# landonclark97/numbotics

Measured on AMD Instinct MI355X. Metric: collision-checked configs/sec, Kinova 7-DoF + obstacles, higher is better.
Workload: dtype f64

## Files before the change

numbotics_amd/csrc/nbk_bf32_spec.hpp:

```cpp

#ifdef NBK_SPEC_NO_ALIGNED
#define NBK_SPEC_ALIGNED 0
#else
#define NBK_SPEC_ALIGNED 1
#endif
#ifdef NBK_SPEC_NO_QREG
#define NBK_SPEC_QREG 0
#else
#define NBK_SPEC_QREG 1
#endif
#ifdef NBK_SPEC_DIAG_NO_WORLD
#define NBK_SPEC_WORLD 0
#else
#define NBK_SPEC_WORLD 1
#endif
#ifdef NBK_SPEC_DIAG_NO_RR
#define NBK_SPEC_RR 0
#else
#define NBK_SPEC_RR 1
#endif
#ifdef NBK_SPEC_DIAG_NO_ENQUEUE
#define NBK_SPEC_ENQUEUE 0
#else
#define NBK_SPEC_ENQUEUE 1
#endif

#define NBK_SPEC_DEV __device__ __forceinline__
#define NBK_SPEC_INLINE __attribute__((always_inline))

namespace nbk_spec {

using namespace nbk;
enum { K_BOX = 2, K_HULL = 4, K_PLANE = 5 };
enum { JK_PRISMATIC = 4 };

template <int V> struct IC { static constexpr int value = V; };
template <int B, int E, class F> NBK_SPEC_DEV void sfor(F&& f) {
    if constexpr (B < E) { f(IC<B>{}); sfor<B + 1, E>(f); }
}

template <class Spec> struct SpecRoute {
    const int* __restrict__ vp_cls;
    NBK_SPEC_DEV int cls(unsigned p) const { return vp_cls[p]; }
    NBK_SPEC_DEV int base(int c) const { return Spec::cls_base[c]; }
    NBK_SPEC_DEV int groups(int c) const { return Spec::cls_groups[c]; }
};

template <class Spec>
NBK_SPEC_DEV void broad_f32_spec(const double* __restrict__ q, long long B, const float* __restrict__ ftb, const float* __restrict__ tab,
                                 unsigned long long* __restrict__ mask_bits, unsigned char* __restrict__ mask_bytes,
                                 unsigned long long* __restrict__ q_count, unsigned long long* __restrict__ q_items, unsigned long long cap,
                                 unsigned char* ovf, const int* __restrict__ vp_cls) {
    constexpr int S = Spec::S, SB = Spec::SB, NQ = Spec::NQ, J = Spec::J, W = Spec::W;
    constexpr FTabOffsets FO = ftab_offsets(W);
    extern __shared__ double lds[];
    const int lane = threadIdx.x;
    const long long base = (long long)blockIdx.x * WAVE;
    double* lds_raw = lds;
    constexpr int qrows = NQ > (SB + 2) / 2 ? NQ : (SB + 2) / 2;
    constexpr int qcap = qrows * (WAVE * 2);
    static_assert(qcap >= BQ_CAP && qcap >= S * WAVE, "the q slab must hold the general stage's queue and one unrolled block's items");
    unsigned* lds_queue = reinterpret_cast<unsigned*>(lds_raw);
    if (base >= B) return;
    const int rows_i = (int)((B - base) < WAVE ? (B - base) : WAVE);
    const bool active = lane < rows_i;
    constexpr bool QREG = NBK_SPEC_QREG != 0 && NQ <= 8;
    double qd[QREG ? NQ : 1];
    if constexpr (QREG) {
        const double* row = q + (base + (active ? lane : 0)) * NQ;
#pragma unroll
        for (int j = 0; j < NQ; ++j) qd[j] = row[j];
    } else {
        stage_plain_rows(q, base, rows_i, NQ, lds_raw, lane);
        __syncthreads();
    }
    auto qat = [&](int j) NBK_SPEC_INLINE { if constexpr (QREG) return qd[j]; else return lds_raw[lane * NQ + j]; };
    int hit = 0;
#pragma unroll
    for (int j = 0; j < NQ; ++j) hit = hit || !(__builtin_fabs(qat(j)) <= 1.7976931348623157e308);
    float cxa[SB], cya[SB], cza[SB];
#pragma unroll
    for (int i = 0; i < SB; ++i) { cxa[i] = 0.0f; cya[i] = 0.0f; cza[i] = 0.0f; }
    float rmax = Spec::f_reach, qabs = 0.0f;
    float qv[J];
#pragma unroll
    for (int k = 0; k < J; ++k) { qv[k] = (float)qat(Spec::qcol[k]); qabs += __builtin_fabsf(qv[k]); }
    XfP T;
    {
        const float* bp = ftb + Spec::f_base;
#pragma unroll
        for (int k = 0; k < 3; ++k) { T.Rc[k] = V2f{bp[k], bp[4 + k]}; T.R2[k] = bp[8 + k]; }
        T.tc = V2f{bp[3], bp[7]}; T.t2 = bp[11];
    }
    auto shapes = [&](auto K) NBK_SPEC_INLINE {
        constexpr int k = decltype(K)::value;
        sfor<Spec::sh_begin[k], Spec::sh_begin[k + 1]>([&](auto SH) NBK_SPEC_INLINE {
            constexpr int sh = decltype(SH)::value;
            const float tl0 = ftb[Spec::f_tl + 3 * sh], tl1 = ftb[Spec::f_tl + 3 * sh + 1], tl2 = ftb[Spec::f_tl + 3 * sh + 2];
            const V2f cp = fma2(T.Rc[2], splat2(tl2), fma2(T.Rc[1], splat2(tl1), fma2(T.Rc[0], splat2(tl0), T.tc)));
            const float c2 = __builtin_fmaf(T.R2[2], tl2, __builtin_fmaf(T.R2[1], tl1, __builtin_fmaf(T.R2[0], tl0, T.t2)));
            cxa[sh] = cp.x; cya[sh] = cp.y; cza[sh] = c2;
            rmax = __builtin_fmaxf(rmax, __builtin_fmaxf(__builtin_fabsf(cp.x), __builtin_fmaxf(__builtin_fabsf(cp.y), __builtin_fabsf(c2))));
        });
    };
    shapes(IC<0>{});
    sfor<0, J>([&](auto K) NBK_SPEC_INLINE {
        constexpr int k = decltype(K)::value;
        constexpr int kind = Spec::jkind[k];
        float s = 0.0f, c = 0.0f;
        if constexpr (kind != JK_PRISMATIC) sincos_f(qv[k], s, c);
        if constexpr (kind <= 2) {
            const JPk jp = *reinterpret_cast<const JPk*>(ftb + Spec::f_pk + 20 * k);
            joint_apply_axis_p<kind>(jp, T, s, c, T);
        } else {
            joint_apply_gen_p(ftb + Spec::f_rot + 27 * k, ftb + Spec::f_trans + 3 * k, ftb + Spec::f_slide + 3 * k, T, qv[k], s, c, T);
        }
        shapes(IC<k + 1>{});
    });
    const float e2 = 2.0f * rmax * __builtin_fmaf(2.4e-7f, qabs, Spec::f_eps);
    if constexpr (!QREG) __syncthreads();
    int qn = 0;
    const SpecRoute<Spec> route{vp_cls};
    const float* wbx_all = tab + FO.wbx;
    if (__builtin_amdgcn_ballot_w64(!(e2 <= Spec::f_e2max)) == 0ull) {
        sfor<0, NBK_SPEC_WORLD ? Spec::NW : 0>([&](auto WI) NBK_SPEC_INLINE {
            constexpr int wi = decltype(WI)::value;
            constexpr int w = Spec::wl[wi];
            constexpr int wk = Spec::wk[wi];
            const float* wc = ftb + Spec::f_wc + 18 * w;
            if constexpr (wk == K_BOX || wk == K_HULL) {
                const float* wb = wbx_all + w * 96;
                const float* ob = ftb + Spec::f_wobb + 6 * w;
                int cwv[SB];
                int acc_c = 0, acc_h = 0;
                sfor<0, SB / 2>([&](auto I) NBK_SPEC_INLINE {
                    constexpr int i = decltype(I)::value;
                    cwv[2 * i] = 0; cwv[2 * i + 1] = 0;
                    if constexpr (Spec::wpair(wi, 2 * i) >= 0 || Spec::wpair(wi, 2 * i + 1) >= 0) {
                        const V2f dx = V2f{cxa[2 * i], cxa[2 * i + 1]} - splat2(wc[0]);
                        const V2f dy = V2f{cya[2 * i], cya[2 * i + 1]} - splat2(wc[1]);
                        const V2f dz = V2f{cza[2 * i], cza[2 * i + 1]} - splat2(wc[2]);
                        V2i cand, certh;
                        if constexpr (wk == K_BOX) box_slot2<NBK_SPEC_ALIGNED != 0 && Spec::wbox_aligned[wi] != 0>(dx, dy, dz, wc, wb + 12 * i, cand, certh);
                        else hull_slot2(dx, dy, dz, wc, ob, wb + 12 * i, cand, certh);
                        cwv[2 * i] = cand.x; cwv[2 * i + 1] = cand.y;
                        acc_c |= cand.x | cand.y;
                        acc_h |= certh.x | certh.y;
                    }
                });
                hit = hit || (acc_h < 0);
                const bool live = active && !hit;
                if (NBK_SPEC_ENQUEUE && __builtin_amdgcn_ballot_w64(acc_c < 0 && live) != 0ull) {
                    queue_room(S * WAVE, qcap, route, lds_queue, qn, base, q_count, q_items, cap, lane, ovf);
                    sfor<0, S>([&](auto A) NBK_SPEC_INLINE {
                        constexpr int a = decltype(A)::value;
                        if constexpr (Spec::wpair(wi, a) >= 0) enqueue_lanes(cwv[a] < 0 && live, (unsigned)Spec::wpair(wi, a), lds_queue, qn, lane);
                    });
                }
            } else {
                const Row16f wkey2r = *reinterpret_cast<const Row16f*>(tab + FO.wkey2 + w * 16);
                const Row16f wcertr = *reinterpret_cast<const Row16f*>(tab + FO.wcert + w * 16);
                const Row16f wkeyr = *reinterpret_cast<const Row16f*>(tab + FO.wkey + w * 16);
                const int* tab_wp = reinterpret_cast<const int*>(tab + FO.wp);
                bool c[SB];
                bool ch = false, anyc = false;
                sfor<0, S>([&](auto A) NBK_SPEC_INLINE {
                    constexpr int a = decltype(A)::value;
                    c[a] = false;
                    if constexpr (Spec::wpair(wi, a) >= 0) {
                        if constexpr (wk == K_PLANE) {
                            if (tab_wp[w * 16 + a] >= 0) plane_slot1(cxa[a] - wc[0], cya[a] - wc[1], cza[a] - wc[2], wc, wkey2r.v[a], wcertr.v[a], c[a], ch);
                        } else {
                            if (wkeyr.v[a] >= 0.0f) sphere_slot1(cxa[a] - wc[0], cya[a] - wc[1], cza[a] - wc[2], wkey2r.v[a], wcertr.v[a], c[a], ch);
                        }
                        anyc = anyc || c[a];
                    }
                });
                hit = hit || ch;
                const bool live = active && !hit;
                if (NBK_SPEC_ENQUEUE && __builtin_amdgcn_ballot_w64(anyc && live) != 0ull) {
                    queue_room(S * WAVE, qcap, route, lds_queue, qn, base, q_count, q_items, cap, lane, ovf);
                    sfor<0, S>([&](auto A) NBK_SPEC_INLINE {
                        constexpr int a = decltype(A)::value;
                        if constexpr (Spec::wpair(wi, a) >= 0) enqueue_lanes(c[a] && live, (unsigned)Spec::wpair(wi, a), lds_queue, qn, lane);
                    });
                }
            }
        });
        if constexpr (Spec::rr_any && NBK_SPEC_RR != 0) {
            sfor<0, S - 1>([&](auto A) NBK_SPEC_INLINE {
                constexpr int a = decltype(A)::value;
                if constexpr (Spec::row_slots(a) > 0) {
                    const Row16f nk = *reinterpret_cast<const Row16f*>(tab + FO.rneg + a * 16);
                    const V2f ax2 = V2f{cxa[a], cxa[a]}, ay2 = V2f{cya[a], cya[a]}, az2 = V2f{cza[a], cza[a]};
                    V2f ev[SB / 2];
                    int acc_e = 0;
                    sfor<(a + 1) / 2, SB / 2>([&](auto I) NBK_SPEC_INLINE {
                        constexpr int i = decltype(I)::value;
                        if constexpr (Spec::rr_group(a, i)) {
                            ev[i] = slot_e2(ax2 - V2f{cxa[2 * i], cxa[2 * i + 1]}, ay2 - V2f{cya[2 * i], cya[2 * i + 1]},
                                            az2 - V2f{cza[2 * i], cza[2 * i + 1]}, V2f{nk.v[2 * i], nk.v[2 * i + 1]});
                            const V2i ei = __builtin_bit_cast(V2i, ev[i]);
                            acc_e |= ei.x | ei.y;
                        }
                    });
                    if (__builtin_amdgcn_ballot_w64(acc_e < 0 && active && !hit) != 0ull) {
                        const Row16f nd = *reinterpret_cast<const Row16f*>(tab + FO.rnd + a * 16);
                        int acc_f = 0;
                        sfor<(a + 1) / 2, SB / 2>([&](auto I) NBK_SPEC_INLINE {
                            constexpr int i = decltype(I)::value;
                            if constexpr (Spec::rr_group(a, i)) {
                                const V2i fi = __builtin_bit_cast(V2i, ev[i] + V2f{nd.v[2 * i], nd.v[2 * i + 1]});
                                acc_f |= fi.x | fi.y;
                            }
                        });
                        hit = hit || (acc_f < 0);
                        const bool live = active && !hit;
                        if (NBK_SPEC_ENQUEUE) queue_room(Spec::row_slots(a) * WAVE, qcap, route, lds_queue, qn, base, q_count, q_items, cap, lane, ovf);
                        sfor<NBK_SPEC_ENQUEUE ? a + 1 : S, S>([&](auto Bb) NBK_SPEC_INLINE {
                            constexpr int b = decltype(Bb)::value;
                            if constexpr (Spec::rr_p(a, b) >= 0) {
                                const V2i ei = __builtin_bit_cast(V2i, ev[b / 2]);
                                enqueue_lanes(((b % 2) ? ei.y : ei.x) < 0 && live, (unsigned)Spec::rr_p(a, b), lds_queue, qn, lane);
                            }
                        });
                    }
                }
            });
        }
    } else {
        const bool cert_ok = e2 <= Spec::f_e2max;
        bool certh = false;
        const float* tab_wkey = tab + FO.wkey; const float* tab_wtc = tab + FO.wtc; const float* tab_wcert = tab + FO.wcert;
        const float* tab_wcin = tab + FO.wcin; const float* tab_rho = tab + FO.rho;
        const int* tab_wp = reinterpret_cast<const int*>(tab + FO.wp);
        const int* tab_rp = reinterpret_cast<const int*>(tab + FO.rp);
        const float* tab_rkey = tab + FO.rkey; const float* tab_rcert = tab + FO.rcert;
        sfor<0, Spec::NW>([&](auto WI) NBK_SPEC_INLINE {
            constexpr int wi = decltype(WI)::value;
            constexpr int w = Spec::wl[wi];
            constexpr int wk = Spec::wk[wi];
            const float* wc = ftb + Spec::f_wc + 18 * w;
            unsigned long long bits = 0ull;
            sfor<0, S>([&](auto A) NBK_SPEC_INLINE {
                constexpr int a = decltype(A)::value;
                if constexpr (Spec::wpair(wi, a) >= 0) {
                    const float dx = cxa[a] - wc[0], dy = cya[a] - wc[1], dz = cza[a] - wc[2];
                    if constexpr (wk == K_PLANE) {
                        if (tab_wp[w * 16 + a] >= 0)
                            bits |= plane_slot_gen(dx, dy, dz, wc, tab_wkey[w * 16 + a], tab_rho[a], e2, tab_wcert[w * 16 + a], certh) ? (1ull << a) : 0ull;
                    } else if constexpr (wk == K_BOX) {
                        if (tab_wkey[w * 16 + a] >= 0.0f)
                            bits |= box_slot_gen(dx, dy, dz, wc, tab_wkey[w * 16 + a], tab_wtc[w * 16 + a], tab_rho[a], e2, tab_wcin[w * 16 + a],
                                                 certh, hit) ? (1ull << a) : 0ull;
                    } else {
                        if (tab_wkey[w * 16 + a] >= 0.0f)
                            bits |= other_slot_gen(dx, dy, dz, wc, ftb + Spec::f_wobb + 6 * w, wk == K_HULL, tab_wkey[w * 16 + a], tab_wtc[w * 16 + a],
                                                   tab_rho[a], e2, tab_wcert[w * 16 + a], certh) ? (1ull << a) : 0ull;
                    }
                }
            });
            hit = hit || (cert_ok && certh);
            if (!active || hit) bits = 0ull;
            drain_bits(bits, PairTab{tab_wp + w * 16}, route, lds_queue, qn, base, q_count, q_items, cap, lane, ovf);
        });
        if constexpr (Spec::rr_any) {
            sfor<0, S - 1>([&](auto A) NBK_SPEC_INLINE {
                constexpr int a = decltype(A)::value;
                unsigned long long bits = 0ull;
                sfor<a + 1, S>([&](auto Bb) NBK_SPEC_INLINE {
                    constexpr int b = decltype(Bb)::value;
                    if constexpr (Spec::rr_p(a, b) >= 0) {
                        bits |= robot_slot_gen(cxa[a] - cxa[b], cya[a] - cya[b], cza[a] - cza[b], tab_rkey[a * 16 + b], e2, tab_rcert[a * 16 + b], certh)
                                    ? (1ull << b) : 0ull;
                    }
                });
                hit = hit || (cert_ok && certh);
                if (!active || hit) bits = 0ull;
                drain_bits(bits, PairTab{tab_rp + a * 16}, route, lds_queue, qn, base, q_count, q_items, cap, lane, ovf);
            });
        }
    }
    if (qn > 0) flush_items_r(route, lds_queue, qn, base, q_count, q_items, cap, lane, ovf);
    write_mask(hit != 0, active, base, lane, mask_bits, mask_bytes);
}

}

#ifndef NBK_SPEC_WAVES
#define NBK_SPEC_WAVES 5
#endif
extern "C" __global__ __launch_bounds__(64, NBK_SPEC_WAVES) void k_broad_f32_spec(
        const double* __restrict__ q, long long B, const float* __restrict__ ftb, const float* __restrict__ tab,
        unsigned long long* __restrict__ mask_bits, unsigned char* __restrict__ mask_bytes, unsigned long long* __restrict__ q_count,
        unsigned long long* __restrict__ q_items, unsigned long long cap, unsigned char* ovf, const int* __restrict__ vp_cls) {
    nbk_spec::broad_f32_spec<Spec>(q, B, ftb, tab, mask_bits, mask_bytes, q_count, q_items, cap, ovf, vp_cls);
}
```

numbotics_amd/csrc/nbk_tables.hpp:

```cpp
#pragma once

namespace nbk {

enum : unsigned {
    D_JOINTS = 1,
    D_CHAIN = 2,
    D_RSHAPES = 4,
    D_WSHAPES = 8,
    D_HULL_VERTS = 16,
    D_HULL_PLANES = 32,
    D_PAIRS = 64,
    D_MOTION = D_JOINTS | D_RSHAPES | D_HULL_VERTS | D_PAIRS,
    D_ALL = 127
};

static int32_t desc_check(const nbk_model_desc* d, unsigned parts) {
    if (d == nullptr) return NBK_ERR_INVALID;
    const int J = d->n_joints, S = d->n_rshapes, W = d->n_wshapes, P = d->n_pairs, H = d->n_hulls;
    if (d->n_q < 0 || J < 0 || S < 0 || W < 0 || P < 0 || H < 0) return NBK_ERR_INVALID;
    if (J > NBK_MAX_JOINTS || d->n_q > NBK_MAX_DOF) return NBK_ERR_UNSUPPORTED;
    if (parts & D_HULL_PLANES) parts |= D_HULL_VERTS;
    if ((parts & D_HULL_VERTS) && H > 0) {
        if (d->hull_vert_begin == nullptr || d->hull_verts == nullptr || d->hull_vert_begin[0] != 0) return NBK_ERR_INVALID;
        for (int h = 0; h < H; ++h) if (d->hull_vert_begin[h + 1] <= d->hull_vert_begin[h]) return NBK_ERR_INVALID;
// ... 178 lines not shown
        else if (par < 0) t.load[k] = -1;
        else {
            if (t.save[par] < 0) t.save[par] = t.slots++;
            t.load[k] = t.save[par];
        }
    }
}

static void order_shapes(const nbk_model_desc* d, ModelTables& t) {
    const int J = d->n_joints, S = d->n_rshapes, W = d->n_wshapes;
    t.begin.assign(J + 2, 0);
    for (int f = -1; f < J; ++f) {
        t.begin[f + 1] = (int)t.order.size();
        for (int s = 0; s < S; ++s) if (d->rshape_frame[s] == f) t.order.push_back(s);
    }
    t.begin[J + 1] = (int)t.order.size();
    t.rs_kind.assign(S, 0); t.rs_row.assign(S, 0);
    t.rs_local.assign(12 * (size_t)S, 0.0); t.rs_core.assign(6 * (size_t)S, 0.0);
    t.rs_hull.assign(S > 0 ? S : 1, -1); t.ws_hull.assign(W > 0 ? W : 1, -1);
    t.rs_frame.assign(S > 0 ? S : 1, -1); t.rs_mask.assign(S > 0 ? S : 1, 0u);
    t.frame_mask = frame_masks(d);
    for (int i = 0; i < S; ++i) {
        const int s = t.order[i];
        int kind;
        robot_core_host(d, s, kind, &t.rs_core[6 * i]);
        if (kind == K_HULL) t.rs_hull[i] = (int)d->rshape_param[4 * s];
        t.rs_kind[i] = kind;
        t.rs_row[i] = t.rows;
        t.rows += host_core_rows(kind);
        memcpy(&t.rs_local[12 * i], d->rshape_local + 12 * s, 12 * sizeof(double));
        t.rs_frame[i] = d->rshape_frame[s];
        t.rs_mask[i] = t.rs_frame[i] >= 0 ? t.frame_mask[t.rs_frame[i]] : 0u;
    }
    t.ws_kind.assign(W, 0); t.ws_core.assign(18 * (size_t)W, 0.0); t.ws_center.assign(3 * (size_t)W, 0.0);
    for (int w = 0; w < W; ++w) {
        double cc[6];  int kind;
        core_params(d->wshape_type[w], d->wshape_param + 4 * w, kind, cc);
        cc[5] = 0.0;
        if (kind == K_HULL) {
            const int h = (int)d->wshape_param[4 * w];
            cc[5] = hull_bound_radius(d->hull_verts + 3 * (size_t)d->hull_vert_begin[h], d->hull_vert_begin[h + 1] - d->hull_vert_begin[h]);
            t.ws_hull[w] = h;
        }
        t.ws_kind[w] = kind;
        t.world_hulls = t.world_hulls || kind == K_HULL;
        const double* T = d->wshape_pose + 12 * w;
        double* o = &t.ws_core[18 * w];
        o[0] = T[3]; o[1] = T[7]; o[2] = T[11];
        for (int j = 0; j < 3; ++j) { o[3 + 3 * j] = T[j]; o[4 + 3 * j] = T[4 + j]; o[5 + 3 * j] = T[8 + j]; }
        if (kind == K_PLANE) { o[9] = d->wshape_param[4 * w]; o[10] = d->wshape_param[4 * w + 1]; o[11] = d->wshape_param[4 * w + 2]; }
        o[12] = cc[0]; o[13] = cc[1]; o[14] = cc[2]; o[15] = cc[3]; o[16] = cc[4];
        o[17] = host_bound_radius(kind, cc);
        t.ws_center[3 * w] = o[0]; t.ws_center[3 * w + 1] = o[1]; t.ws_center[3 * w + 2] = o[2];
    }
}

static void pair_tables(const nbk_model_desc* d, ModelTables& t) {
    const int S = d->n_rshapes, P = d->n_pairs;
    std::vector<int> new_index(S);
    for (int i = 0; i < S; ++i) new_index[t.order[i]] = i;
    t.pa.assign(P, 0); t.pb.assign(P, 0); t.pu.assign(P, 0); t.pdev.assign(P > 0 ? P : 1, 0);
    std::vector<int> vcls(P), vorder(P), refA(P), refB(P);
    for (int p = 0; p < P; ++p) {
        t.pa[p] = new_index[d->pair_a[p]];
        t.pb[p] = d->pair_b[p] < S ? new_index[d->pair_b[p]] : d->pair_b[p];
        t.pu[p] = p;
        t.pdev[t.pu[p]] = p;
        refA[p] = t.pa[p];
        refB[p] = t.pb[p] < S ? t.pb[p] : ~(t.pb[p] - S);
        const int ka = t.kind_of(refA[p]), kb = t.kind_of(refB[p]);
        const bool a_ps = (ka == K_POINT || ka == K_SEG), b_ps = (kb == K_POINT || kb == K_SEG);
        if (kb == K_PLANE) vcls[p] = 0;
        else if (ka == K_HULL || kb == K_HULL) vcls[p] = 2;
        else if ((a_ps && b_ps) || ka == K_POINT || kb == K_POINT) vcls[p] = 1;
        else vcls[p] = 2;
    }
    int cur = 0;
    for (int c = 0; c < 3; ++c)
        for (int p = 0; p < P; ++p)
            if (vcls[p] == c) { vorder[cur++] = p; if (c == 0) ++t.n_plane; if (c == 1) ++t.n_closed; }
    t.vp_tab.assign(4 * (size_t)P, 0); t.vp_canon.assign(2 * (size_t)P, 0); t.vp_cst.assign(4 * (size_t)P, 0.0);
    for (int i = 0; i < P; ++i) {
        const int p = vorder[i];
        const int ka = t.kind_of(refA[p]), kb = t.kind_of(refB[p]);
        t.vp_tab[4 * i] = refA[p]; t.vp_tab[4 * i + 1] = refB[p]; t.vp_tab[4 * i + 2] = vcls[p]; t.vp_tab[4 * i + 3] = p;
        const bool swap = ka > kb;
        t.vp_canon[2 * i] = swap ? refB[p] : refA[p];
        t.vp_canon[2 * i + 1] = swap ? refA[p] : refB[p];
        const double* ca = t.core_of(refA[p]);
        const double* cb = t.core_of(refB[p]);
        t.vp_cst[4 * i] = ca[4]; t.vp_cst[4 * i + 1] = cb[4];
        t.vp_cst[4 * i + 2] = host_bound_radius(ka, ca);
        t.vp_cst[4 * i + 3] = host_bound_radius(kb, cb);
        const int k0 = ka < kb ? ka : kb, k1 = ka < kb ? kb : ka;
        const bool closed = k1 != K_HULL && (k0 == K_POINT || ((k0 == K_POINT || k0 == K_SEG) && (k1 == K_POINT || k1 == K_SEG)));
        if (k1 != K_PLANE && !closed && (ca[4] != 0.0 || cb[4] != 0.0)) t.margins_zero = false;
        if (k1 != K_PLANE && !closed) { t.gjk_margins.push_back(ca[4]); t.gjk_margins.push_back(cb[4]); if (k1 == K_HULL) t.gjk_any_hull = true; }
    }
}

static void broad_order(const nbk_model_desc* d, ModelTables& t) {
    const int P = d->n_pairs;
    t.bq_tab.assign(4 * (size_t)(P > 0 ? P : 1), 0);
    int cur_b = 0;
    for (int cat = 0; cat < 4; ++cat)
        for (int i = 0; i < P; ++i) {
            const int ra = t.vp_tab[4 * i], rb = t.vp_tab[4 * i + 1];
            const int c = rb >= 0 ? 1 : (t.ws_kind[~rb] == K_PLANE ? 0 : (t.ws_kind[~rb] == K_BOX ? 3 : 2));
            if (c != cat) continue;
            t.bq_tab[4 * cur_b] = 3 * ra;
            t.bq_tab[4 * cur_b + 1] = rb >= 0 ? 3 * rb : ~rb;
            t.bq_tab[4 * cur_b + 2] = i;
            t.bq_tab[4 * cur_b + 3] = cat;
            ++cur_b;
        }
}

static double pair_reach_bound(const nbk_model_desc* d, const ModelTables& t, int j, const double* poses) {
    const int cat = t.bq_tab[4 * j + 3], a = t.bq_tab[4 * j] / 3, w = t.bq_tab[4 * j + 1], i = t.bq_tab[4 * j + 2];
    if (cat == 1 || !(t.reach[a] < INFINITY)) return -INFINITY;
    const double* T = poses + 12 * (size_t)w;
    const double c[3] = {T[3], T[7], T[11]}, b0[3] = {d->base_pose[3], d->base_pose[7], d->base_pose[11]};
    return world_reach_bound(cat == 0, c, d->wshape_param + 4 * (size_t)w, b0, t.reach[a], t.vp_cst[4 * i + 2], t.vp_cst[4 * i + 3]);
}

static void static_reach(const nbk_model_desc* d, ModelTables& t) {
    const int J = d->n_joints, S = d->n_rshapes, P = d->n_pairs;
    t.bq_static.assign((size_t)(P > 0 ? P : 1), -INFINITY);
    t.reach.assign(S > 0 ? S : 1, 0.0);
    for (int i = 0; i < S; ++i) {
        const int f = t.rs_frame[i];
        double r = 0.0;
        bool unbounded = false;
        if (f >= 0)
            for (int k = 0; k < J; ++k)
                if ((t.frame_mask[f] >> k) & 1u) {
                    if (d->joint_type[k] == NBK_PRISMATIC) unbounded = true;
                    r += std::sqrt(d->joint_trans[3 * k] * d->joint_trans[3 * k] + d->joint_trans[3 * k + 1] * d->joint_trans[3 * k + 1] +
                                   d->joint_trans[3 * k + 2] * d->joint_trans[3 * k + 2]);
                }
        const double lx = t.rs_local[12 * i + 3], ly = t.rs_local[12 * i + 7], lz = t.rs_local[12 * i + 11];
        r += std::sqrt(lx * lx + ly * ly + lz * lz);
        t.reach[i] = unbounded ? INFINITY : r * (1.0 + 1e-12) + 1e-12;
    }
    for (int j = 0; j < P; ++j) t.bq_static[j] = pair_reach_bound(d, t, j, d->wshape_pose);
}

static void compile_geometry(const nbk_model_desc* d, ModelTables& t) {
    plan_frames(d, t);
    order_shapes(d, t);
    pair_tables(d, t);
    broad_order(d, t);
    static_reach(d, t);
}

static int32_t check_limits(const nbk_model_desc* d, ModelTables& t) {
    const int S = d->n_rshapes, W = d->n_wshapes, P = d->n_pairs;
    if (3 * S >= 65536 || W >= 65536 || P >= (1 << 20)) return NBK_ERR_UNSUPPORTED;
    t.lds_broad_ok = lds_broad_ok(d->n_q, t.slots, S, P, W);
    if (!t.lds_broad_ok && S > 16) return NBK_ERR_UNSUPPORTED;
    t.parked_ok = ValidityLds(d->n_q, t.rows > d->n_q ? t.rows : d->n_q, t.slots).fits();
    if (S <= 16 && !broad_f32_ok(d->n_q, t.slots, S)) return NBK_ERR_UNSUPPORTED;
    if (P >= (1 << 26)) return NBK_ERR_UNSUPPORTED;
    return NBK_OK;
}

template <class T>
static void pack_joint_rot(const double* M, int joint_kind, T* out) {
    const int kz = joint_kind <= 2 ? joint_kind : 0;
    const int u = (kz + 1) % 3, v = (kz + 2) % 3;
    for (int r = 0; r < 3; ++r) {
        out[2 * r] = (T)M[18 + 3 * r + u]; out[2 * r + 1] = (T)M[18 + 3 * r + v];
        out[6 + 2 * r] = (T)M[9 + 3 * r + u]; out[6 + 2 * r + 1] = (T)M[9 + 3 * r + v];
        out[12 + r] = (T)M[3 * r + kz];
    }
}

static int32_t joint_tables(const nbk_model_desc* d, ModelTables& t) {
    const int J = d->n_joints;
    t.jrot.assign(d->joint_rot, d->joint_rot + 27 * (size_t)J); t.jtrans.assign(d->joint_trans, d->joint_trans + 3 * (size_t)J);
    for (double& v : t.jrot) v += 0.0;  for (double& v : t.jtrans) v += 0.0;
    t.joint_kind.assign(J > 0 ? J : 1, JK_GENERIC);
    t.joint_pk.assign(22 * (size_t)(J > 0 ? J : 1), 0.0);
    for (int k = 0; k < J; ++k) {
        const double* Mk = &t.jrot[27 * (size_t)k];
        if (d->joint_type[k] == NBK_PRISMATIC) {
            bool zero = true;
            for (int e = 9; e < 27; ++e) zero = zero && Mk[e] == 0.0;
            if (!zero) { snprintf(g_err, sizeof(g_err), "prismatic joint %d: M1 / M2 of joint_rot must be zero", k); return NBK_ERR_INVALID; }
            t.joint_kind[k] = JK_PRISMATIC;
        } else {
            for (int kz = 0; kz < 3; ++kz) {
                const int u = (kz + 1) % 3, v = (kz + 2) % 3;
                bool ok = d->joint_slide[3 * k] == 0.0 && d->joint_slide[3 * k + 1] == 0.0 && d->joint_slide[3 * k + 2] == 0.0;
                for (int r = 0; r < 3; ++r)
                    ok = ok && Mk[9 + 3 * r + kz] == 0.0 && Mk[18 + 3 * r + kz] == 0.0 && Mk[3 * r + u] == 0.0 && Mk[3 * r + v] == 0.0;
                if (ok) { t.joint_kind[k] = kz; break; }
            }
        }
        double* jp = &t.joint_pk[22 * (size_t)k];
        pack_joint_rot(Mk, t.joint_kind[k], jp);
        for (int r = 0; r < 3; ++r) { jp[15 + r] = t.jtrans[3 * k + r]; jp[18 + r] = d->joint_axis[3 * k + r]; }
    }
    motion_tables(d, t.frame_mask, t.mh);
    return NBK_OK;
}

static void queue_groups(const nbk_model_desc* d, ModelTables& t) {
    const int P = d->n_pairs;
    t.vp_info.assign(4 * (size_t)(P > 0 ? P : 1), 0);
    t.vp_cls.assign((size_t)(P > 0 ? P : 1), 3);
    for (int i = 0; i < P; ++i) {
        const int ra = t.vp_canon[2 * i], rb = t.vp_canon[2 * i + 1];
        t.vp_info[4 * i] = ra; t.vp_info[4 * i + 1] = rb;
        t.vp_info[4 * i + 2] = ra >= 0 ? (int)t.rs_mask[ra] : 0;
        t.vp_info[4 * i + 3] = rb >= 0 ? (int)t.rs_mask[rb] : 0;
        const int ka = t.kind_of(ra), kb = t.kind_of(rb);
        t.vp_cls[i] = (ka == K_BOX && kb == K_BOX) ? 0 : ((ka == K_BOX && kb == K_CYL) ? 1 : ((ka == K_CYL && kb == K_CYL) ? 2 : 3));
        t.cls_count[t.vp_cls[i]] += 1;
    }
    int used = 0, nonempty = 0;
    for (int c = 0; c < 4; ++c) if (t.cls_count[c] > 0) ++nonempty;
    const int spare = NSUB - nonempty;
    for (int c = 0; c < 4; ++c)
        if (t.cls_count[c] > 0) { t.cls_groups[c] = 1 + (int)((long long)spare * t.cls_count[c] / (P > 0 ? P : 1)); used += t.cls_groups[c]; }
    int big = 0;
    for (int c = 1; c < 4; ++c) if (t.cls_count[c] > t.cls_count[big]) big = c;
    if (P > 0) t.cls_groups[big] += NSUB - used;
    for (int c = 1; c < 4; ++c) t.cls_base[c] = t.cls_base[c - 1] + t.cls_groups[c - 1];
}

static void float_tables(const nbk_model_desc* d, const double* world_radius, ModelTables& t) {
    const int J = d->n_joints, S = d->n_rshapes, W = d->n_wshapes, H = d->n_hulls;
    t.hull_obb.assign(6 * (size_t)(H > 0 ? H : 1), 0.0);
    for (int h = 0; h < H; ++h) {
        const double* v = d->hull_verts + 3 * (size_t)d->hull_vert_begin[h];
        const int n = d->hull_vert_begin[h + 1] - d->hull_vert_begin[h];
        double lo[3] = {v[0], v[1], v[2]}, hi[3] = {v[0], v[1], v[2]};
        for (int k = 1; k < n; ++k)
            for (int j = 0; j < 3; ++j) { lo[j] = std::min(lo[j], v[3 * k + j]); hi[j] = std::max(hi[j], v[3 * k + j]); }
        for (int j = 0; j < 3; ++j) { t.hull_obb[6 * h + j] = 0.5 * (lo[j] + hi[j]); t.hull_obb[6 * h + 3 + j] = 0.5 * (hi[j] - lo[j]) * (1.0 + 1e-12) + 1e-300; }
    }
    std::vector<float>& ftab = t.ftab;
    double freach = 0.0;
    for (int k = 0; k < J; ++k) for (int e = 0; e < 27; ++e) ftab.push_back((float)d->joint_rot[27 * k + e]);
    t.f_trans = (int)ftab.size();
    for (int k = 0; k < J; ++k) {
        double n2 = 0.0;
        for (int e = 0; e < 3; ++e) { ftab.push_back((float)d->joint_trans[3 * k + e]); n2 += d->joint_trans[3 * k + e] * d->joint_trans[3 * k + e]; }
        freach += std::sqrt(n2);
    }
    t.f_slide = (int)ftab.size();
    for (int k = 0; k < J; ++k) for (int e = 0; e < 3; ++e) ftab.push_back((float)d->joint_slide[3 * k + e]);
    t.f_base = (int)ftab.size();
    double b2 = 0.0;
    for (int e = 0; e < 12; ++e) ftab.push_back((float)d->base_pose[e]);
    for (int i = 0; i < 3; ++i) b2 += d->base_pose[4 * i + 3] * d->base_pose[4 * i + 3];
    freach += std::sqrt(b2);
    t.f_tl = (int)ftab.size();
    double lmax = 0.0;
    for (int i = 0; i < S; ++i) {
        double n2 = 0.0;
        for (int r = 0; r < 3; ++r) { const double v = t.rs_local[12 * i + 4 * r + 3]; ftab.push_back((float)v); n2 += v * v; }
        if (std::sqrt(n2) > lmax) lmax = std::sqrt(n2);
    }
    freach += lmax;
    t.f_wc = (int)ftab.size();
    for (int w = 0; w < W; ++w) {
        double n2 = 0.0;
        for (int e = 0; e < 18; ++e) ftab.push_back((float)t.ws_core[18 * w + e]);
        for (int e = 0; e < 3; ++e) n2 += t.ws_core[18 * w + e] * t.ws_core[18 * w + e];
        if (std::sqrt(n2) > freach) freach = std::sqrt(n2);
    }
    if (world_radius != nullptr && *world_radius > freach) freach = *world_radius;
    t.f_wobb = (int)ftab.size();
    for (int w = 0; w < W; ++w)
        for (int e = 0; e < 6; ++e) {
            const double v = t.ws_hull[w] >= 0 ? t.hull_obb[6 * (size_t)t.ws_hull[w] + e] : 0.0;
            ftab.push_back(e < 3 ? (float)v : (float)v * (1.0f + 2.4e-7f));
        }
    while (ftab.size() % 4 != 0) ftab.push_back(0.0f);
    t.f_pk = (int)ftab.size();
    ftab.resize(ftab.size() + 20 * (size_t)(J > 8 ? J : 8), 0.0f);
    for (int k = 0; k < J; ++k) {
        float* fp = &ftab[t.f_pk + 20 * (size_t)k];
        pack_joint_rot(d->joint_rot + 27 * (size_t)k, t.joint_kind[k], fp);
        for (int e = 0; e < 3; ++e) fp[16 + e] = (float)d->joint_trans[3 * k + e];
    }
    t.f_meta = (int)ftab.size();
    for (int k = 0; k < 8; ++k) {
        const unsigned v = k < J ? ((unsigned)t.joint_kind[k] | ((unsigned)d->joint_qidx[k] << 8)) : 0u;
        float fv; memcpy(&fv, &v, 4);
        ftab.push_back(fv);
    }
    t.f_chain = (J >= 1 && J <= 8 && S <= 16) ? 1 : 0;
    for (int k = 0; k < J && t.f_chain; ++k) if (t.load[k] != (k == 0 ? -1 : -2) || t.save[k] != -1) t.f_chain = 0;
    const double rel = 50.0 * (J + 2) * 16.0 * 5.96e-8;
    t.f_eps = (float)(rel > 1e-4 ? rel : 1e-4);
    t.f_reach = (float)(freach > 1e-3 ? freach : 1e-3);
    t.f_e2max = 2.0f * t.f_reach * (t.f_eps + 2.4e-7f * 64.0f) * (1.0f + 1e-6f);
}

constexpr int SPEC_MAX_WORLD = 2;

static std::string bf32_spec_text(const nbk_model_desc* d, const ModelTables& t, bool movable) {
    const int S = d->n_rshapes, J = d->n_joints, W = d->n_wshapes, P = d->n_pairs;
    if (!t.f_chain || P == 0 || S < 1 || S > 16 || J < 1 || J > 8) return std::string();
    std::vector<int> rrp((size_t)S * S, -1), wlist;
    std::vector<int> wslot_of(W > 0 ? W : 1, -1);
    for (int j = 0; j < P; ++j) {
        const int* bt = &t.bq_tab[4 * j];
        if (bt[3] != 1 && wslot_of[bt[1]] < 0) { wslot_of[bt[1]] = 0; wlist.push_back(bt[1]); }
    }
    std::sort(wlist.begin(), wlist.end());
    if ((int)wlist.size() > SPEC_MAX_WORLD) return std::string();
    const int NW = (int)wlist.size();
    for (int i = 0; i < NW; ++i) wslot_of[wlist[i]] = i;
    std::vector<int> wp((size_t)(NW > 0 ? NW : 1) * S, -1);
    bool rr_any = false;
    for (int j = 0; j < P; ++j) {
        const int* bt = &t.bq_tab[4 * j];
        const int a = bt[0] / 3;
        if (bt[3] == 1) {
            const int b = bt[1] / 3, lo = a < b ? a : b, hi = a < b ? b : a;
            rrp[(size_t)lo * S + hi] = bt[2];
            rr_any = true;
        } else {
            wp[(size_t)wslot_of[bt[1]] * S + a] = bt[2];
        }
    }
    std::string o;
    char buf[512];
    auto add = [&](const char* fmt, auto... v) { snprintf(buf, sizeof(buf), fmt, v...); o += buf; };
    auto arr = [&](const char* name, const std::vector<int>& v) {
        add("    static constexpr int %s[] = {", name);
        for (size_t i = 0; i < v.size(); ++i) add(i ? ", %d" : "%d", v[i]);
        if (v.empty()) o += "-1";
        o += "};\n";
    };
    const int SB = S <= 8 ? 8 : (S <= 12 ? 12 : 16);
    o += "struct Spec {\n";
    add("    static constexpr int S = %d, SB = %d, NQ = %d, J = %d, W = %d, NW = %d;\n", S, SB, d->n_q, J, W, NW);
    arr("jkind", std::vector<int>(t.joint_kind.begin(), t.joint_kind.begin() + J));
    arr("qcol", std::vector<int>(d->joint_qidx, d->joint_qidx + J));
    arr("sh_begin", t.begin);
    add("    static constexpr int f_rot = 0, f_pk = %d, f_tl = %d, f_base = %d, f_wc = %d, f_wobb = %d, f_trans = %d, f_slide = %d;\n",
        t.f_pk, t.f_tl, t.f_base, t.f_wc, t.f_wobb, t.f_trans, t.f_slide);
    add("    static constexpr float f_eps = %af, f_reach = %af, f_e2max = %af;\n", (double)t.f_eps, (double)t.f_reach, (double)t.f_e2max);
    add("    static constexpr bool rr_any = %s;\n", rr_any ? "true" : "false");
    arr("rrp_", rrp);
    std::vector<int> wk;
    for (int w : wlist) wk.push_back(t.ws_kind[w]);
    arr("wl", wlist);
    arr("wk", wk);
    arr("wp_", wp);
    std::vector<int> aligned;
    for (int w : wlist) {
        bool id = !movable && t.ws_kind[w] == K_BOX;
        for (int e = 0; e < 9 && id; ++e) id = t.ftab[t.f_wc + 18 * (size_t)w + 3 + e] == (e % 4 == 0 ? 1.0f : 0.0f);
        aligned.push_back(id ? 1 : 0);
    }
    arr("wbox_aligned", aligned);
    arr("cls_base", std::vector<int>(t.cls_base, t.cls_base + 4));
    std::vector<int> groups(t.cls_groups, t.cls_groups + 4);
    for (int& g : groups) g = g > 0 ? g : 1;
    arr("cls_groups", groups);
    o += "    static constexpr int rr_p(int a, int b) { return a >= 0 && b < S && a < b ? rrp_[a * S + b] : -1; }\n"
         "    static constexpr int wpair(int wi, int a) { return a < S ? wp_[wi * S + a] : -1; }\n"
         "    static constexpr bool rr_group(int a, int i) { return rr_p(a, 2 * i) >= 0 || rr_p(a, 2 * i + 1) >= 0; }\n"
         "    static constexpr int row_slots(int a) { int n = 0; for (int b = a + 1; b < S; ++b) n += rr_p(a, b) >= 0 ? 1 : 0; return n; }\n"
         "};\n";
    return o;
}

static void hull_tables(const nbk_model_desc* d, ModelTables& t) {
    const int S = d->n_rshapes, W = d->n_wshapes, H = d->n_hulls;
    auto inscribed = [&](int kind, const double* cc, int hull) {
        double r = 0.0;
        if (kind == K_BOX) r = std::min(cc[0], std::min(cc[1], cc[2]));
        else if (kind == K_CYL) r = std::min(cc[3], cc[0]);
        else if (kind == K_HULL) {
            const int f0 = d->hull_face_begin[hull], f1 = d->hull_face_begin[hull + 1];
            r = f1 > f0 ? INFINITY : 0.0;
            for (int f = f0; f < f1; ++f) r = std::min(r, d->hull_planes[4 * (size_t)f + 3]);
            r *= (1.0 - 1e-9);
        } else if (kind == K_PLANE) return 0.0;
        if (!(r > 0.0)) r = 0.0;
        return r + cc[4];
    };
    t.rs_in.assign(S > 0 ? S : 1, 0.0); t.ws_in.assign(W > 0 ? W : 1, 0.0);
    for (int i = 0; i < S; ++i) t.rs_in[i] = inscribed(t.rs_kind[i], &t.rs_core[6 * (size_t)i], t.rs_hull[i]);
    for (int w = 0; w < W; ++w) t.ws_in[w] = inscribed(t.ws_kind[w], &t.ws_core[18 * (size_t)w + 12], t.ws_hull[w]);
    t.hull_off.assign(H > 0 ? H : 1, 0);
    for (int h = 0; h < H; ++h) {
        const double* v = d->hull_verts + 3 * (size_t)d->hull_vert_begin[h];
        const int n = d->hull_vert_begin[h + 1] - d->hull_vert_begin[h];
        t.hull_blob.insert(t.hull_blob.end(), &t.hull_obb[6 * h], &t.hull_obb[6 * h] + 6);
        t.hull_off[h] = t.hull_blob.size();
        t.hull_blob.insert(t.hull_blob.end(), v, v + 3 * (size_t)n);
    }
}

static int32_t compile_tables(const nbk_model_desc* d, const double* world_radius, ModelTables& t) {
    compile_geometry(d, t);
    { const int32_t rc = check_limits(d, t); if (rc != NBK_OK) return rc; }
    { const int32_t rc = joint_tables(d, t); if (rc != NBK_OK) return rc; }
    queue_groups(d, t);
    float_tables(d, world_radius, t);
    t.spec = bf32_spec_text(d, t, world_radius != nullptr);
    hull_tables(d, t);
    return NBK_OK;
}

}
```

Baseline: 10.23 billion.

## Constant-fold zero and unit joint/shape coefficients into specialized FK kernels

Classifies each packed joint and shape-offset coefficient on the host as zero, +1, -1 or general, and emits these classes into the generated spec struct. The FK sweep then uses compile-time folded dot products that drop multiplies by zero and turn unit multiplies into adds or subtracts. A wave-uniform ballot on the joint magnitude picks the folded or generic sweep. This shrinks the per-config FK arithmetic in the broad phase, at the cost of two inlined code paths and more code size and register pressure. Treating near-zero coefficients as exact zero relies on bounds checks to keep the error within the existing epsilon margin.

```diff
diff --git a/numbotics_amd/csrc/nbk_bf32_spec.hpp b/numbotics_amd/csrc/nbk_bf32_spec.hpp
--- a/numbotics_amd/csrc/nbk_bf32_spec.hpp
+++ b/numbotics_amd/csrc/nbk_bf32_spec.hpp
@@ -8,6 +8,14 @@
 #define NBK_SPEC_QREG 0
 #else
 #define NBK_SPEC_QREG 1
+#endif
+#ifdef NBK_SPEC_NO_FOLD
+#define NBK_SPEC_FOLD 0
+#else
+#define NBK_SPEC_FOLD 1
+#endif
+#ifndef NBK_SPEC_FOLD_PARTS
+#define NBK_SPEC_FOLD_PARTS 3
 #endif
 #ifdef NBK_SPEC_DIAG_NO_WORLD
 #define NBK_SPEC_WORLD 0
@@ -45,6 +53,62 @@
     NBK_SPEC_DEV int base(int c) const { return Spec::cls_base[c]; }
     NBK_SPEC_DEV int groups(int c) const { return Spec::cls_groups[c]; }
 };
+
+constexpr float FOLD_QMAX = 0x1p20f;
+enum { FC_GEN = 0, FC_ZERO = 1, FC_ONE = 2, FC_NEG = 3 };
+
+NBK_SPEC_DEV V2f fold_mul(V2f a, float k) { return a * splat2(k); }
+NBK_SPEC_DEV V2f fold_mul(V2f a, V2f k) { return a * k; }
+NBK_SPEC_DEV float fold_mul(float a, float k) { return a * k; }
+NBK_SPEC_DEV V2f fold_fma(V2f a, float k, V2f acc) { return fma2(a, splat2(k), acc); }
+NBK_SPEC_DEV V2f fold_fma(V2f a, V2f k, V2f acc) { return fma2(a, k, acc); }
+NBK_SPEC_DEV float fold_fma(float a, float k, float acc) { return __builtin_fmaf(a, k, acc); }
+
+template <int CL, bool EMPTY, class T, class K> NBK_SPEC_DEV T fold_term(T a, K k, T acc) {
+    if constexpr (CL == FC_ZERO) return acc;
+    else if constexpr (CL == FC_ONE) { if constexpr (EMPTY) return a; else return a + acc; }
+    else if constexpr (CL == FC_NEG) { if constexpr (EMPTY) return -a; else return acc - a; }
+    else { if constexpr (EMPTY) return fold_mul(a, k); else return fold_fma(a, k, acc); }
+}
+template <int C0, int C1, int C2, bool HAS, class T, class K> NBK_SPEC_DEV T fold_dot3(T a0, T a1, T a2, K k0, K k1, K k2, T init) {
+    constexpr bool e0 = !HAS, e1 = e0 && C0 == FC_ZERO, e2 = e1 && C1 == FC_ZERO;
+    return fold_term<C2, e2>(a2, k2, fold_term<C1, e1>(a1, k1, fold_term<C0, e0>(a0, k0, init)));
+}
+template <int C2, int C1> NBK_SPEC_DEV float fold_l(float s, float c, float m2, float m1) {
+    if constexpr (C2 == FC_ZERO && C1 == FC_ZERO) return 0.0f;
+    else if constexpr (C2 == FC_ZERO) return -fold_term<C1, true>(c, m1, 0.0f);
+    else if constexpr (C1 == FC_ZERO) return fold_term<C2, true>(s, m2, 0.0f);
+    else return __builtin_fmaf(s, m2, -(c * m1));
+}
+template <class C> struct FoldL {
+    float x[3], y[3];
+    static constexpr int z(int i) { return C::at(i) == FC_ZERO && C::at(6 + i) == FC_ZERO ? FC_ZERO : FC_GEN; }
+    static constexpr int pz(int r) { return z(2 * r) == FC_ZERO && z(2 * r + 1) == FC_ZERO ? FC_ZERO : FC_GEN; }
+    NBK_SPEC_DEV FoldL(const JPk& jp, float s, float c) {
+        x[0] = fold_l<C::at(0), C::at(6)>(s, c, jp.m2p[0], jp.m1p[0]);  y[0] = fold_l<C::at(1), C::at(7)>(s, c, jp.m2p[1], jp.m1p[1]);
+        x[1] = fold_l<C::at(2), C::at(8)>(s, c, jp.m2p[2], jp.m1p[2]);  y[1] = fold_l<C::at(3), C::at(9)>(s, c, jp.m2p[3], jp.m1p[3]);
+        x[2] = fold_l<C::at(4), C::at(10)>(s, c, jp.m2p[4], jp.m1p[4]); y[2] = fold_l<C::at(5), C::at(11)>(s, c, jp.m2p[5], jp.m1p[5]);
+    }
+};
+template <int KZ, class C>
+NBK_SPEC_DEV void joint_apply_axis_fold(const JPk& jp, const XfP& P, float s, float c, XfP& o) {
+    constexpr int U = (KZ + 1) % 3, V = (KZ + 2) % 3;
+    using Z = FoldL<C>;
+    const Z L(jp, s, c);
+    const V2f z2 = V2f{0.0f, 0.0f};
+    const V2f cu = fold_dot3<Z::z(0), Z::z(2), Z::z(4), false>(P.Rc[0], P.Rc[1], P.Rc[2], L.x[0], L.x[1], L.x[2], z2);
+    const V2f cv = fold_dot3<Z::z(1), Z::z(3), Z::z(5), false>(P.Rc[0], P.Rc[1], P.Rc[2], L.y[0], L.y[1], L.y[2], z2);
+    const V2f ck = fold_dot3<C::at(12), C::at(13), C::at(14), false>(P.Rc[0], P.Rc[1], P.Rc[2], jp.mk[0], jp.mk[1], jp.mk[2], z2);
+    const V2f r2 = fold_dot3<Z::pz(0), Z::pz(1), Z::pz(2), false>(splat2(P.R2[0]), splat2(P.R2[1]), splat2(P.R2[2]), V2f{L.x[0], L.y[0]},
+                                                                  V2f{L.x[1], L.y[1]}, V2f{L.x[2], L.y[2]}, z2);
+    const float r2k = fold_dot3<C::at(12), C::at(13), C::at(14), false>(P.R2[0], P.R2[1], P.R2[2], jp.mk[0], jp.mk[1], jp.mk[2], 0.0f);
+    const V2f tc = fold_dot3<C::at(15), C::at(16), C::at(17), true>(P.Rc[0], P.Rc[1], P.Rc[2], jp.toff[0], jp.toff[1], jp.toff[2], P.tc);
+    const float t2 = fold_dot3<C::at(15), C::at(16), C::at(17), true>(P.R2[0], P.R2[1], P.R2[2], jp.toff[0], jp.toff[1], jp.toff[2], P.t2);
+    o.Rc[U] = cu; o.Rc[V] = cv; o.Rc[KZ] = ck;
+    o.R2[U] = r2.x; o.R2[V] = r2.y; o.R2[KZ] = r2k;
+    o.tc = tc; o.t2 = t2;
+}
+template <class Spec, int K> struct PkClass { static constexpr int at(int i) { return Spec::fc_pk[18 * K + i]; } };
 
 template <class Spec>
 NBK_SPEC_DEV void broad_f32_spec(const double* __restrict__ q, long long B, const float* __restrict__ ftb, const float* __restrict__ tab,
@@ -85,38 +149,57 @@
     float qv[J];
 #pragma unroll
     for (int k = 0; k < J; ++k) { qv[k] = (float)qat(Spec::qcol[k]); qabs += __builtin_fabsf(qv[k]); }
-    XfP T;
-    {
-        const float* bp = ftb + Spec::f_base;
-#pragma unroll
-        for (int k = 0; k < 3; ++k) { T.Rc[k] = V2f{bp[k], bp[4 + k]}; T.R2[k] = bp[8 + k]; }
-        T.tc = V2f{bp[3], bp[7]}; T.t2 = bp[11];
-    }
-    auto shapes = [&](auto K) NBK_SPEC_INLINE {
-        constexpr int k = decltype(K)::value;
-        sfor<Spec::sh_begin[k], Spec::sh_begin[k + 1]>([&](auto SH) NBK_SPEC_INLINE {
-            constexpr int sh = decltype(SH)::value;
-            const float tl0 = ftb[Spec::f_tl + 3 * sh], tl1 = ftb[Spec::f_tl + 3 * sh + 1], tl2 = ftb[Spec::f_tl + 3 * sh + 2];
-            const V2f cp = fma2(T.Rc[2], splat2(tl2), fma2(T.Rc[1], splat2(tl1), fma2(T.Rc[0], splat2(tl0), T.tc)));
-            const float c2 = __builtin_fmaf(T.R2[2], tl2, __builtin_fmaf(T.R2[1], tl1, __builtin_fmaf(T.R2[0], tl0, T.t2)));
-            cxa[sh] = cp.x; cya[sh] = cp.y; cza[sh] = c2;
-            rmax = __builtin_fmaxf(rmax, __builtin_fmaxf(__builtin_fabsf(cp.x), __builtin_fmaxf(__builtin_fabsf(cp.y), __builtin_fabsf(c2))));
+    auto sweep = [&](auto FOLD) NBK_SPEC_INLINE {
+        constexpr bool fold = decltype(FOLD)::value != 0;
+        constexpr bool fold_joints = fold && (NBK_SPEC_FOLD_PARTS & 1) != 0, fold_shapes = fold && (NBK_SPEC_FOLD_PARTS & 2) != 0;
+        XfP T;
+        {
+            const float* bp = ftb + Spec::f_base;
+#pragma unroll
+            for (int k = 0; k < 3; ++k) { T.Rc[k] = V2f{bp[k], bp[4 + k]}; T.R2[k] = bp[8 + k]; }
+            T.tc = V2f{bp[3], bp[7]}; T.t2 = bp[11];
+        }
+        auto shapes = [&](auto K) NBK_SPEC_INLINE {
+            constexpr int k = decltype(K)::value;
+            sfor<Spec::sh_begin[k], Spec::sh_begin[k + 1]>([&](auto SH) NBK_SPEC_INLINE {
+                constexpr int sh = decltype(SH)::value;
+                const float tl0 = ftb[Spec::f_tl + 3 * sh], tl1 = ftb[Spec::f_tl + 3 * sh + 1], tl2 = ftb[Spec::f_tl + 3 * sh + 2];
+                V2f cp;
+                float c2;
+                if constexpr (fold_shapes) {
+                    constexpr int c0 = Spec::fc_tl[3 * sh], c1 = Spec::fc_tl[3 * sh + 1], c2c = Spec::fc_tl[3 * sh + 2];
+                    cp = fold_dot3<c0, c1, c2c, true>(T.Rc[0], T.Rc[1], T.Rc[2], tl0, tl1, tl2, T.tc);
+                    c2 = fold_dot3<c0, c1, c2c, true>(T.R2[0], T.R2[1], T.R2[2], tl0, tl1, tl2, T.t2);
+                } else {
+                    cp = fma2(T.Rc[2], splat2(tl2), fma2(T.Rc[1], splat2(tl1), fma2(T.Rc[0], splat2(tl0), T.tc)));
+                    c2 = __builtin_fmaf(T.R2[2], tl2, __builtin_fmaf(T.R2[1], tl1, __builtin_fmaf(T.R2[0], tl0, T.t2)));
+                }
+                cxa[sh] = cp.x; cya[sh] = cp.y; cza[sh] = c2;
+                rmax = __builtin_fmaxf(rmax, __builtin_fmaxf(__builtin_fabsf(cp.x), __builtin_fmaxf(__builtin_fabsf(cp.y), __builtin_fabsf(c2))));
+            });
+        };
+        shapes(IC<0>{});
+        sfor<0, J>([&](auto K) NBK_SPEC_INLINE {
+            constexpr int k = decltype(K)::value;
+            constexpr int kind = Spec::jkind[k];
+            float s = 0.0f, c = 0.0f;
+            if constexpr (kind != JK_PRISMATIC) sincos_f(qv[k], s, c);
+            if constexpr (kind <= 2) {
+                const JPk jp = *reinterpret_cast<const JPk*>(ftb + Spec::f_pk + 20 * k);
+                if constexpr (fold_joints) joint_apply_axis_fold<kind, PkClass<Spec, k>>(jp, T, s, c, T);
+                else joint_apply_axis_p<kind>(jp, T, s, c, T);
+            } else {
+                joint_apply_gen_p(ftb + Spec::f_rot + 27 * k, ftb + Spec::f_trans + 3 * k, ftb + Spec::f_slide + 3 * k, T, qv[k], s, c, T);
+            }
+            shapes(IC<k + 1>{});
         });
     };
-    shapes(IC<0>{});
-    sfor<0, J>([&](auto K) NBK_SPEC_INLINE {
-        constexpr int k = decltype(K)::value;
-        constexpr int kind = Spec::jkind[k];
-        float s = 0.0f, c = 0.0f;
-        if constexpr (kind != JK_PRISMATIC) sincos_f(qv[k], s, c);
-        if constexpr (kind <= 2) {
-            const JPk jp = *reinterpret_cast<const JPk*>(ftb + Spec::f_pk + 20 * k);
-            joint_apply_axis_p<kind>(jp, T, s, c, T);
-        } else {
-            joint_apply_gen_p(ftb + Spec::f_rot + 27 * k, ftb + Spec::f_trans + 3 * k, ftb + Spec::f_slide + 3 * k, T, qv[k], s, c, T);
-        }
-        shapes(IC<k + 1>{});
-    });
+    if constexpr (NBK_SPEC_FOLD != 0 && (NBK_SPEC_FOLD_PARTS & 3) != 0 && Spec::fc_any != 0) {
+        if (__builtin_amdgcn_ballot_w64(!(qabs < FOLD_QMAX)) == 0ull) sweep(IC<1>{});
+        else sweep(IC<0>{});
+    } else {
+        sweep(IC<0>{});
+    }
     const float e2 = 2.0f * rmax * __builtin_fmaf(2.4e-7f, qabs, Spec::f_eps);
     if constexpr (!QREG) __syncthreads();
     int qn = 0;
diff --git a/numbotics_amd/csrc/nbk_tables.hpp b/numbotics_amd/csrc/nbk_tables.hpp
--- a/numbotics_amd/csrc/nbk_tables.hpp
+++ b/numbotics_amd/csrc/nbk_tables.hpp
@@ -504,6 +504,12 @@
 }
 
 constexpr int SPEC_MAX_WORLD = 2;
+
+constexpr float FOLD_ZERO_REL = 0x1p-40f;
+static int fold_class(float v, float zero_below) {
+    if (std::fabs(v) <= zero_below) return 1;
+    return v == 1.0f ? 2 : (v == -1.0f ? 3 : 0);
+}
 
 static std::string bf32_spec_text(const nbk_model_desc* d, const ModelTables& t, bool movable) {
     const int S = d->n_rshapes, J = d->n_joints, W = d->n_wshapes, P = d->n_pairs;
@@ -563,6 +569,23 @@
         aligned.push_back(id ? 1 : 0);
     }
     arr("wbox_aligned", aligned);
+    bool fold_ok = t.f_reach <= 0x1p20f;
+    for (int e = 0; e < 27 * J; ++e) fold_ok = fold_ok && std::fabs(t.ftab[e]) <= 2.0f;
+    for (int e = 0; e < 3 * J; ++e) fold_ok = fold_ok && std::fabs(t.ftab[t.f_trans + e]) <= 0x1p20f && std::fabs(t.ftab[t.f_slide + e]) <= 0x1p20f;
+    for (int e = 0; e < 12; ++e) fold_ok = fold_ok && std::fabs(t.ftab[t.f_base + e]) <= (e % 4 == 3 ? 0x1p20f : 2.0f);
+    for (int e = 0; e < 3 * S; ++e) fold_ok = fold_ok && std::fabs(t.ftab[t.f_tl + e]) <= 0x1p20f;
+    const float zr = FOLD_ZERO_REL, zt = FOLD_ZERO_REL * t.f_reach;
+    std::vector<int> fc_pk, fc_tl;
+    bool fold_any = false;
+    for (int k = 0; k < J; ++k)
+        for (int e = 0; e < 18; ++e) {
+            fc_pk.push_back(fold_ok ? (e < 15 ? fold_class(t.ftab[t.f_pk + 20 * (size_t)k + e], zr) : fold_class(t.ftab[t.f_pk + 20 * (size_t)k + e + 1], zt)) : 0);
+            fold_any = fold_any || (t.joint_kind[k] <= 2 && fc_pk.back() != 0);
+        }
+    for (int e = 0; e < 3 * S; ++e) { fc_tl.push_back(fold_ok ? fold_class(t.ftab[t.f_tl + e], zt) : 0); fold_any = fold_any || fc_tl.back() != 0; }
+    add("    static constexpr int fc_any = %d;\n", fold_any ? 1 : 0);
+    arr("fc_pk", fc_pk);
+    arr("fc_tl", fc_tl);
     arr("cls_base", std::vector<int>(t.cls_base, t.cls_base + 4));
     std::vector<int> groups(t.cls_groups, t.cls_groups + 4);
     for (int& g : groups) g = g > 0 ? g : 1;
```

Measured after the change: 11.00 billion, median of 6. 1.08x the previous value.
